# BillyXYB/TransEditor

Measured on AMD Instinct MI355X. Metric: 256x256 images/sec/GPU, G+D fwd+bwd, batch 16; 1/2/4/8-GPU scaling, higher is better.
Workload: dtype f32

## Files before the change

include/te_hip.h:

```cpp
#ifndef TE_HIP_H
#define TE_HIP_H

#include <stdint.h>

#ifdef __cplusplus
extern "C" {
#endif

#define TE_ABI_VERSION 3

#define TE_ERR_NULL -1
#define TE_ERR_SHAPE -2
#define TE_ERR_UNSUPPORTED -3
#define TE_ERR_WORKSPACE -4

typedef void* te_stream_t;

int te_version(void);
const char* te_last_error_string(void);
const char* te_arch(void);

int te_bias_act_f32(float* out, const float* x, const float* b, const float* ref, int act, int grad,
                    float alpha, float scale, int64_t size_x, int64_t step_b, int64_t size_b,
                    te_stream_t stream);
// ... 130 lines not shown
                             const float* residual, int I, int J, int K, int64_t sai, int64_t sak, int64_t sbk, int64_t sbj,
                             float alpha, float beta, int act, te_stream_t stream);

int te_minibatch_stddev_fwd_f32(float* y, const float* x, int B, int group, int C, int HW, float eps, te_stream_t stream);
int te_minibatch_stddev_bwd_f32(float* gx, const float* gy, const float* x, int B, int group, int C, int HW, float eps,
                                te_stream_t stream);

int te_layer_norm_supported(int64_t R, int N);
int te_layer_norm_fwd_f32(float* y, float* stats, const float* x, int64_t R, int N, float eps, te_stream_t stream);
int te_layer_norm_bwd_f32(float* gx, const float* g, const float* y, const float* stats, int64_t R, int N, te_stream_t stream);

int te_pixel_norm_supported(int64_t B, int D, int C);
int te_pixel_norm_fwd_f32(float* y, float* r, const float* x, int64_t B, int D, int C, float eps, te_stream_t stream);
int te_pixel_norm_bwd_f32(float* gx, const float* g, const float* y, const float* r, int64_t B, int D, int C, te_stream_t stream);

int te_small_gemm_batched_f32(float* c, const float* a, const float* b, const float* bias, int nz, int64_t za, int64_t zc,
                              int64_t zb, int64_t zbias, const int64_t* b_tab, const int64_t* bias_tab, int I, int J, int K,
                              int64_t sai, int64_t sak, int64_t sbk, int64_t sbj, int64_t sci, int64_t scj, float alpha,
                              float beta, int act, te_stream_t stream);

int te_demod_fwd_f32(float* d, float* wsq, const float* w, const float* s, float wscale, float eps, int B, int Co, int Ci,
                     int T, te_stream_t stream);
int te_demod_bwd_f32(float* gw, float* gs, const float* gd, const float* d, const float* w, const float* wsq,
                     const float* s, float wscale, int B, int Co, int Ci, int T, int accumulate, te_stream_t stream);

int te_mt_adam_f32(const int64_t* table, const int32_t* chunks, int n_tensors, int n_chunks, int chunk_elems, double lr,
                   double beta1, double beta2, double eps, int step, te_stream_t stream);
int te_mt_ema_f32(const int64_t* table, const int32_t* chunks, int n_tensors, int n_chunks, int chunk_elems, double decay,
                  te_stream_t stream);

int te_chan_scale_f32(float* out, const float* x, const float* s, int64_t rows, int64_t hw, te_stream_t stream);
int te_chan_dot_f32(float* out, const float* a, const float* b, int64_t rows, int64_t hw, te_stream_t stream);

int te_lpips_stem_fwd_f32(float* out, const float* x, const float* w, const float* b, int N, int H, int W, te_stream_t stream);
int te_lpips_stem_dgrad_f32(float* gx, const float* g, const float* y1, const float* w, int N, int H, int W, te_stream_t stream);
int te_maxpool2_fwd_f32(float* out, const float* x, int64_t planes, int H, int W, te_stream_t stream);
int te_maxpool2_bwd_f32(float* gx, const float* g, const float* x, int64_t planes, int H, int W, te_stream_t stream);
int te_lpips_normalize_f32(float* out, const float* x, int N, int C, int64_t HW, te_stream_t stream);
int te_lpips_head_blocks(int64_t HW);
int te_lpips_head_fwd_f32(float* partial, const float* f, const float* t, const float* w, int N, int Nt, int C, int64_t HW,
                          te_stream_t stream);
int te_lpips_dist_f32(float* d, const float* const* partial, const int64_t* hw, int L, int N, te_stream_t stream);
int te_lpips_head_bwd_f32(float* gf, const float* gin, const float* gd, const float* f, const float* t, const float* w, int N, int Nt,
                          int C, int64_t HW, int relu_mask, te_stream_t stream);
int te_lpips_pair_head_fwd_f32(float* partial, const float* f, const float* w, int N, int C, int64_t HW, te_stream_t stream);
int te_crop_resize_bilinear_f32(float* out, const float* img, int B, int H, int W, int y0, int x0, int hc, int wc, int h, int w,
                                te_stream_t stream);

int64_t te_noise_reg_ws_floats(const int* sizes, int n, int B);
int te_noise_reg_fwd_f32(float* loss, float* ws, float* const* maps, const int* sizes, int n, int B, te_stream_t stream);
int te_noise_reg_bwd_f32(float* const* grads, float* tws, const float* gloss, const float* ws, float* const* maps, const int* sizes,
                         int n, int B, te_stream_t stream);
int te_noise_normalize_f32(float* const* maps, const int* sizes, int n, int B, te_stream_t stream);

int64_t te_prdc_ws_bytes(int N, int M, int D, int k);
int te_row_sqnorm_f32(float* out, const float* x, int N, int D, te_stream_t stream);
int te_prdc_knn_f32(float* r2, const float* x, const float* nx, int N, int D, int k, void* ws, te_stream_t stream);
int te_prdc_counts_f32(int32_t* col_count, int32_t* row_any, float* row_min, const float* x, const float* nx, const float* rr2,
                       const float* y, const float* ny, const float* rf2, int N, int M, int D, void* ws, te_stream_t stream);

int te_vgg_stem_fwd_f32(float* out, const float* x, const float* w, const float* b, int N, int H, int W, te_stream_t stream);
int te_adaptive_avgpool_f32(float* out, const float* x, int64_t planes, int H, int W, int OH, int OW, te_stream_t stream);
int te_fc_stream_splits(int J, int K);
int64_t te_fc_stream_ws_bytes(int64_t I, int J, int K);
int te_fc_stream_f32(float* c, float* ws, const float* a, const float* w, const float* bias, int64_t I, int J, int K, int act,
                     te_stream_t stream);
// ... 20 lines not shown
```

transeditor_amd/_lib.py:

```python
import ctypes as C
import os

import torch

_HERE = os.path.dirname(os.path.abspath(__file__))
LIB_PATH = os.path.join(_HERE, 'libte_hip.so')
_lib = None

CONV_3X3, CONV_T2, CONV_S2, CONV_1X1, CONV_3X3W, CONV_3X3W6, CONV_S2S6, CONV_T2S6, CONV_1X1S6 = 0, 1, 2, 3, 4, 5, 6, 7, 8
(PACK_FWD, PACK_DGRAD, PACK_SWAP, PACK_WFWD, PACK_WDGRAD, PACK_W6FWD, PACK_W6DGRAD, PACK_S6FWD, PACK_S6SWAP, PACK_T6FWD,
 PACK_T6SWAP, PACK_P6FWD, PACK_P6DGRAD) = range(13)

_P, _I, _L, _F = C.c_void_p, C.c_int, C.c_int64, C.c_float
_SIGNATURES = {
    'te_version': (C.c_int, []),
    'te_last_error_string': (C.c_char_p, []),
    'te_arch': (C.c_char_p, []),
    'te_bias_act_f32': (C.c_int, [_P, _P, _P, _P, _I, _I, _F, _F, _L, _L, _L, _P]),
    'te_bias_act_f16': (C.c_int, [_P, _P, _P, _P, _I, _I, _F, _F, _L, _L, _L, _P]),
    'te_bias_act_f64': (C.c_int, [_P, _P, _P, _P, _I, _I, _F, _F, _L, _L, _L, _P]),
    'te_bias_act_bwd_ws_floats': (C.c_int64, [_L, _L, _L]),
    'te_bias_act_bwd_f32': (C.c_int, [_P, _P, _P, _P, _P, _F, _F, _L, _L, _L, _P]),
    'te_bias_act_bwd_rgb_supported': (C.c_int, [_L, _L, _L]),
    'te_bias_act_bwd_rgb_f32': (C.c_int, [_P, _P, _P, _P, _P, _P, _P, _P, _F, _F, _F, _L, _L, _L, _P]),
# ... 29 lines not shown
    'te_wgrad_group_f32': (C.c_int, [_P, _P, _P, _I, _I, _I, _I, _I, _I, _I, _I, _P]),
    'te_wgrad_reduce_ws_floats': (C.c_int64, [_I, _I, _I, _I, _I, _I, _I, _I]),
    'te_wgrad_reduce_f32': (C.c_int, [_P, _P, _P, _P, _P, _P, _F, _P, _P, _I, _I, _I, _I, _I, _P]),
    'te_rgb_supported': (C.c_int, [_I, _I, _I]),
    'te_rgb_fwd_f32': (C.c_int, [_P, _P, _P, _P, _P, _F, _I, _I, _I, _P]),
    'te_rgb_dgrad_f32': (C.c_int, [_P, _P, _P, _P, _F, _I, _I, _I, _P]),
    'te_rgb_wgrad_sum_f32': (C.c_int, [_P, _P, _P, _I, _I, _I, _I, _P]),
    'te_rgb_expand_f32': (C.c_int, [_P, _P, _P, _P, _I, _F, _I, _I, _I, _P]),
    'te_rgb_wgrad_slab_count': (C.c_int, [_I, _I, _I]),
    'te_rgb_wgrad_f32': (C.c_int, [_P, _P, _P, _I, _I, _I, _I, _P]),
    'te_blur_actgrad_tiles': (C.c_int, [_I] * 8),
    'te_blur_actgrad_f32': (C.c_int, [_P, _P, _P, _P, _P, _L, _I, _I, _I, _I, _I, _I, _I, _I, _F, _F, _P]),
    'te_blur_gradact_f32': (C.c_int, [_P, _P, _P, _P, _P, _L, _I, _I, _I, _I, _I, _I, _I, _I, _F, _F, _P]),
    'te_small_gemm_f32': (C.c_int, [_P, _P, _P, _P, _P, _P, _P, _F, _I, _I, _I, _L, _L, _L, _L, _F, _F, _I, _P]),
    'te_small_gemm_batched_f32': (C.c_int, [_P, _P, _P, _P, _I, _L, _L, _L, _L, _P, _P, _I, _I, _I, _L, _L, _L, _L, _L, _L,
                                             _F, _F, _I, _P]),
    'te_layer_norm_supported': (C.c_int, [_L, _I]),
    'te_layer_norm_fwd_f32': (C.c_int, [_P, _P, _P, _L, _I, _F, _P]),
    'te_layer_norm_bwd_f32': (C.c_int, [_P, _P, _P, _P, _L, _I, _P]),
    'te_pixel_norm_supported': (C.c_int, [_L, _I, _I]),
    'te_pixel_norm_fwd_f32': (C.c_int, [_P, _P, _P, _L, _I, _I, _F, _P]),
    'te_pixel_norm_bwd_f32': (C.c_int, [_P, _P, _P, _P, _L, _I, _I, _P]),
    'te_demod_fwd_f32': (C.c_int, [_P, _P, _P, _P, _F, _F, _I, _I, _I, _I, _P]),
    'te_demod_bwd_f32': (C.c_int, [_P, _P, _P, _P, _P, _P, _P, _F, _I, _I, _I, _I, _I, _P]),
    'te_attn_fwd_f32': (C.c_int, [_P, _P, _P, _P, _P, _F, _I, _I, _I, _I, _I, _P]),
    'te_attn_bwd_f32': (C.c_int, [_P, _P, _P, _P, _P, _P, _P, _P, _P, _F, _I, _I, _I, _I, _I, _P]),
    'te_small_gemm_splitk_f32': (C.c_int, [_P, _P, _P, _I, _P, _P, _P, _P, _I, _I, _I, _L, _L, _L, _L, _F, _F, _I, _P]),
    'te_minibatch_stddev_fwd_f32': (C.c_int, [_P, _P, _I, _I, _I, _I, _F, _P]),
    'te_minibatch_stddev_bwd_f32': (C.c_int, [_P, _P, _P, _I, _I, _I, _I, _F, _P]),
    'te_mt_adam_f32': (C.c_int, [_P, _P, _I, _I, _I, C.c_double, C.c_double, C.c_double, C.c_double, _I, _P]),
    'te_mt_ema_f32': (C.c_int, [_P, _P, _I, _I, _I, C.c_double, _P]),
    'te_chan_scale_f32': (C.c_int, [_P, _P, _P, _L, _L, _P]),
    'te_chan_dot_f32': (C.c_int, [_P, _P, _P, _L, _L, _P]),
    'te_lpips_stem_fwd_f32': (C.c_int, [_P, _P, _P, _P, _I, _I, _I, _P]),
    'te_lpips_stem_dgrad_f32': (C.c_int, [_P, _P, _P, _P, _I, _I, _I, _P]),
    'te_maxpool2_fwd_f32': (C.c_int, [_P, _P, _L, _I, _I, _P]),
    'te_maxpool2_bwd_f32': (C.c_int, [_P, _P, _P, _L, _I, _I, _P]),
    'te_lpips_normalize_f32': (C.c_int, [_P, _P, _I, _I, _L, _P]),
    'te_lpips_head_blocks': (C.c_int, [_L]),
    'te_lpips_head_fwd_f32': (C.c_int, [_P, _P, _P, _P, _I, _I, _I, _L, _P]),
    'te_lpips_dist_f32': (C.c_int, [_P, _P, _P, _I, _I, _P]),
    'te_lpips_head_bwd_f32': (C.c_int, [_P, _P, _P, _P, _P, _P, _I, _I, _I, _L, _I, _P]),
    'te_lpips_pair_head_fwd_f32': (C.c_int, [_P, _P, _P, _I, _I, _L, _P]),
    'te_crop_resize_bilinear_f32': (C.c_int, [_P, _P, _I, _I, _I, _I, _I, _I, _I, _I, _I, _P]),
    'te_noise_reg_ws_floats': (C.c_int64, [_P, _I, _I]),
    'te_noise_reg_fwd_f32': (C.c_int, [_P, _P, _P, _P, _I, _I, _P]),
    'te_noise_reg_bwd_f32': (C.c_int, [_P, _P, _P, _P, _P, _P, _I, _I, _P]),
    'te_noise_normalize_f32': (C.c_int, [_P, _P, _I, _I, _P]),
    'te_prdc_ws_bytes': (C.c_int64, [_I, _I, _I, _I]),
    'te_row_sqnorm_f32': (C.c_int, [_P, _P, _I, _I, _P]),
    'te_prdc_knn_f32': (C.c_int, [_P, _P, _P, _I, _I, _I, _P, _P]),
    'te_prdc_counts_f32': (C.c_int, [_P, _P, _P, _P, _P, _P, _P, _P, _P, _I, _I, _I, _P, _P]),
    'te_vgg_stem_fwd_f32': (C.c_int, [_P, _P, _P, _P, _I, _I, _I, _P]),
    'te_adaptive_avgpool_f32': (C.c_int, [_P, _P, _L, _I, _I, _I, _I, _P]),
    'te_fc_stream_splits': (C.c_int, [_I, _I]),
    'te_fc_stream_ws_bytes': (C.c_int64, [_L, _I, _I]),
    'te_fc_stream_f32': (C.c_int, [_P, _P, _P, _P, _P, _L, _I, _I, _I, _P]),
    'te_fid_moments_ws_bytes': (C.c_int64, [_L, _I]),
    'te_fid_moments_f64': (C.c_int, [_P, _P, _P, _P, _L, _I, _I, _P]),
    'te_fid_finalize_f64': (C.c_int, [_P, _P, _P, _P, _L, _I, _P]),
    'te_gram_f32': (C.c_int, [_P, _P, _I, _I, _P]),
    'te_svm_smo_f64': (C.c_int, [_P, _P, _P, _P, _P, _I, C.c_double, C.c_double, _L, _P]),
    'te_svm_coef_f32': (C.c_int, [_P, _P, _P, _P, _I, _I, _P]),
    'te_conv2d_f32': (C.c_int, [_P, _P, _P, _P] + [_I] * 13 + [_P]),
    'te_pool3_f32': (C.c_int, [_P, _P, _I, _I, _I, _I, _I, _I, _I, _P]),
    'te_resize_bilinear_f32': (C.c_int, [_P, _P, _L, _I, _I, _I, _I, _P]),
# ... 546 lines not shown
                                 _ptr(gsim.contiguous()) if gsim is not None else None, _ptr(q), _ptr(k), _ptr(v),
                                 _ptr(sim), scale, N, groups, M, L, Cn // groups, _stream()), 'te_attn_bwd_f32')
    return gq, gk, gv


def mt_adam(table, chunks, n_tensors, n_chunks, chunk_elems, lr, beta1, beta2, eps, step):
    _on_current_device(table)
    _check(lib().te_mt_adam_f32(table.data_ptr(), chunks.data_ptr(), n_tensors, n_chunks, chunk_elems, lr, beta1, beta2, eps,
                                step, _stream()), 'te_mt_adam_f32')


def mt_ema(table, chunks, n_tensors, n_chunks, chunk_elems, decay):
    _on_current_device(table)
    _check(lib().te_mt_ema_f32(table.data_ptr(), chunks.data_ptr(), n_tensors, n_chunks, chunk_elems, float(decay), _stream()),
           'te_mt_ema_f32')


def chan_scale(x, s):
    x, s = x.contiguous(), s.contiguous()
    rows = x.shape[0] * x.shape[1]
    out = torch.empty_like(x)
    _check(lib().te_chan_scale_f32(_ptr(out), _ptr(x), _ptr(s), rows, x.numel() // max(rows, 1), _stream()), 'te_chan_scale_f32')
    return out


def chan_dot(a, b):
    a, b = a.contiguous(), b.contiguous()
    rows = a.shape[0] * a.shape[1]
    out = torch.empty(a.shape[0], a.shape[1], device=a.device, dtype=a.dtype)
    _check(lib().te_chan_dot_f32(_ptr(out), _ptr(a), _ptr(b), rows, a.numel() // max(rows, 1), _stream()), 'te_chan_dot_f32')
    return out


def lpips_stem_fwd(x, w, b):
    x = x.contiguous()
    N, _, H, W = x.shape
    out = torch.empty(N, 64, H, W, device=x.device, dtype=x.dtype)
    _check(lib().te_lpips_stem_fwd_f32(_ptr(out), _ptr(x), _ptr(w), _ptr(b), N, H, W, _stream()), 'te_lpips_stem_fwd_f32')
    return out


def lpips_stem_dgrad(g, y1, w):
    g = g.contiguous()
    N, _, H, W = g.shape
    gx = torch.empty(N, 3, H, W, device=g.device, dtype=g.dtype)
    _check(lib().te_lpips_stem_dgrad_f32(_ptr(gx), _ptr(g), _ptr(y1), _ptr(w), N, H, W, _stream()), 'te_lpips_stem_dgrad_f32')
    return gx


def maxpool2_fwd(x):
    x = x.contiguous()
    N, Cn, H, W = x.shape
    out = torch.empty(N, Cn, H // 2, W // 2, device=x.device, dtype=x.dtype)
    _check(lib().te_maxpool2_fwd_f32(_ptr(out), _ptr(x), N * Cn, H, W, _stream()), 'te_maxpool2_fwd_f32')
    return out


def maxpool2_bwd(g, x):
    g = g.contiguous()
    N, Cn, H, W = x.shape
    gx = torch.empty_like(x)
    _check(lib().te_maxpool2_bwd_f32(_ptr(gx), _ptr(g), _ptr(x), N * Cn, H, W, _stream()), 'te_maxpool2_bwd_f32')
    return gx


def lpips_normalize(x):
# ... 269 lines not shown
    out = _slice_out(out, c0, B, Co, max(Ho, 0), max(Wo, 0), x, 'conv2d')
    _check(lib().te_conv2d_f32(_ptr(out), _ptr(x), _ptr(w), _ptr(bias), B, Ci, Co, H, W, kh, kw, stride, pad[0], pad[1], out.shape[1],
                               c0, act, _stream()), 'te_conv2d_f32')
    return out


def pool3(x, mode, out=None, c0=0):
    if x.ndim != 4:
        raise RuntimeError(f'te_hip: pool3 expects [B,C,H,W], got {tuple(x.shape)}')
    B, Cn, H, W = x.shape
    Ho, Wo = ((H - 3) // 2 + 1, (W - 3) // 2 + 1) if mode == POOL3_MAX_S2 else (H, W)
    out = _slice_out(out, c0, B, Cn, max(Ho, 0), max(Wo, 0), x, 'pool3')
    _check(lib().te_pool3_f32(_ptr(out), _ptr(x), B, Cn, H, W, mode, out.shape[1], c0, _stream()), 'te_pool3_f32')
    return out


def resize_bilinear(x, OH, OW):
    if x.ndim != 4:
        raise RuntimeError(f'te_hip: resize_bilinear expects [B,C,H,W], got {tuple(x.shape)}')
    x = x.contiguous()
    B, Cn, H, W = x.shape
    out = torch.empty(B, Cn, OH, OW, device=x.device, dtype=x.dtype)
    _check(lib().te_resize_bilinear_f32(_ptr(out), _ptr(x), B * Cn, H, W, OH, OW, _stream()), 'te_resize_bilinear_f32')
    return out


def _install_roctx():
    import functools
    import torch.cuda.nvtx as nvtx
    names = ['bias_act', 'bias_act_bwd', 'upfirdn2d_raw', 'blur_actgrad', 'blur_gradact', 'conv_pack', 'conv_pack2', 'conv_pack_multi', 'conv',
             'wgrad_slabs', 'wgrad_reduce', 'rgb_fwd', 'rgb_dgrad', 'rgb_expand', 'rgb_wgrad_slabs', 'small_gemm',
             'small_gemm_splitk', 'small_gemm_batched', 'minibatch_stddev_fwd', 'minibatch_stddev_bwd',
             'layer_norm_fwd', 'layer_norm_bwd', 'pixel_norm_fwd', 'pixel_norm_bwd', 'demod_fwd', 'demod_from_wsq', 'demod_bwd',
             'attn_fwd', 'attn_bwd', 'mt_adam', 'mt_ema', 'chan_scale', 'chan_dot', 'lpips_stem_fwd', 'lpips_stem_dgrad',
             'maxpool2_fwd', 'maxpool2_bwd', 'lpips_normalize', 'lpips_head_fwd', 'lpips_dist', 'lpips_head_bwd', 'lpips_pair_head_fwd', 'crop_resize_bilinear', 'noise_reg_fwd',
             'noise_reg_bwd', 'noise_normalize_', 'row_sqnorm', 'prdc_knn', 'prdc_counts', 'vgg_stem_fwd', 'adaptive_avgpool', 'fc_stream',
             'fid_moments', 'fid_finalize', 'gram', 'svm_smo', 'svm_coef', 'conv2d', 'pool3', 'resize_bilinear']
    g = globals()

    def wrap(fn, name):
        @functools.wraps(fn)
        def run(*a, **k):
            t = next((x for x in a if torch.is_tensor(x)), None)
            nvtx.range_push(f'te:{name} {tuple(t.shape)}' if t is not None else f'te:{name}')
            try:
                return fn(*a, **k)
            finally:
                nvtx.range_pop()
        return run
    for n in names:
        if n in g:
            g[n] = wrap(g[n], n)


ROCTX = os.environ.get('TE_ROCTX') == '1'
if ROCTX:
    _install_roctx()
```

transeditor_amd/csrc/chanscale.hip:

```cpp
#include "te_common.h"

namespace {

__global__ __launch_bounds__(256) void chan_scale_vec4_kernel(float4* __restrict__ out, const float4* __restrict__ x,
                                                              const float* __restrict__ s, int64_t n4, uint32_t hw4) {
    const int64_t stride = (int64_t)gridDim.x * blockDim.x;
    for (int64_t i = (int64_t)blockIdx.x * blockDim.x + threadIdx.x; i < n4; i += stride) {
        const float sc = s[i / hw4];
        float4 v = x[i];
        v.x *= sc; v.y *= sc; v.z *= sc; v.w *= sc;
        out[i] = v;
    }
}

__global__ __launch_bounds__(256) void chan_scale_flat4_kernel(float4* __restrict__ out, const float4* __restrict__ x,
                                                               const float* __restrict__ s, int64_t n4, int64_t hw) {
    const int64_t stride = (int64_t)gridDim.x * blockDim.x;
    for (int64_t i = (int64_t)blockIdx.x * blockDim.x + threadIdx.x; i < n4; i += stride) {
        const int64_t e = 4 * i, r = e / hw;
        const int left = (int)(hw - (e - r * hw));
        const float s0 = s[r], s1 = left < 4 ? s[r + 1] : s0;
        float4 v = x[i];
        v.x *= s0;
        v.y *= left > 1 ? s0 : s1;
// ... 31 lines not shown
        const float4* b4 = reinterpret_cast<const float4*>(br);
        const int64_t n4 = hw / 4;
        float c0 = 0.f, c1 = 0.f, c2 = 0.f, c3 = 0.f;
        int64_t j = tid;
        for (; j + 768 < n4; j += 1024) {
            const float4 u0 = a4[j], u1 = a4[j + 256], u2 = a4[j + 512], u3 = a4[j + 768];
            const float4 v0 = b4[j], v1 = b4[j + 256], v2 = b4[j + 512], v3 = b4[j + 768];
            c0 += u0.x * v0.x + u0.y * v0.y + u0.z * v0.z + u0.w * v0.w;
            c1 += u1.x * v1.x + u1.y * v1.y + u1.z * v1.z + u1.w * v1.w;
            c2 += u2.x * v2.x + u2.y * v2.y + u2.z * v2.z + u2.w * v2.w;
            c3 += u3.x * v3.x + u3.y * v3.y + u3.z * v3.z + u3.w * v3.w;
        }
        for (; j < n4; j += 256) {
            const float4 u = a4[j], v = b4[j];
            c0 += u.x * v.x + u.y * v.y + u.z * v.z + u.w * v.w;
        }
        acc = (c0 + c1) + (c2 + c3);
    } else {
        float c0 = 0.f, c1 = 0.f;
        int64_t j = tid;
        for (; j + 256 < hw; j += 512) { c0 += ar[j] * br[j]; c1 += ar[j + 256] * br[j + 256]; }
        for (; j < hw; j += 256) c0 += ar[j] * br[j];
        acc = c0 + c1;
    }
#pragma unroll
    for (int off = 32; off > 0; off >>= 1) acc += __shfl_down(acc, off, 64);
    if (lane == 0) part[wid] = acc;
    __syncthreads();
    if (tid == 0) out[r] = (part[0] + part[1]) + (part[2] + part[3]);
}

inline bool aligned16(const void* p) { return (reinterpret_cast<uintptr_t>(p) & 15) == 0; }

}

extern "C" int te_chan_scale_f32(float* out, const float* x, const float* s, int64_t rows, int64_t hw, te_stream_t stream_) {
    TE_REQUIRE(out && x && s, TE_ERR_NULL, "te_chan_scale_f32: NULL pointer");
    TE_REQUIRE(rows >= 0 && hw > 0, TE_ERR_SHAPE, "te_chan_scale_f32: bad dims");
    if (rows == 0) return 0;
    hipStream_t st = (hipStream_t)stream_;
    const int64_t n = rows * hw;
    if (hw % 4 == 0 && aligned16(out) && aligned16(x) && hw / 4 < (int64_t)0xFFFFFFFF) {
        const int grid = (int)std::min<int64_t>(te::cdiv(n / 4, 256), te::kNumCU * 16);
        chan_scale_vec4_kernel<<<grid, 256, 0, st>>>((float4*)out, (const float4*)x, s, n / 4, (uint32_t)(hw / 4));
    } else if (hw >= 4 && n >= 1024 && aligned16(out) && aligned16(x)) {
        const int grid = (int)std::min<int64_t>(te::cdiv(n / 4, 256), te::kNumCU * 16);
        chan_scale_flat4_kernel<<<grid, 256, 0, st>>>((float4*)out, (const float4*)x, s, n / 4, hw);
        if (n % 4) chan_scale_kernel<<<1, 64, 0, st>>>(out, x, s, n, hw, n - n % 4);
    } else {
        const int grid = (int)std::min<int64_t>(te::cdiv(n, 256), te::kNumCU * 16);
        chan_scale_kernel<<<grid, 256, 0, st>>>(out, x, s, n, hw, 0);
    }
    return te::launch_status("te_chan_scale_f32");
}

extern "C" int te_chan_dot_f32(float* out, const float* a, const float* b, int64_t rows, int64_t hw, te_stream_t stream_) {
    TE_REQUIRE(out && a && b, TE_ERR_NULL, "te_chan_dot_f32: NULL pointer");
    TE_REQUIRE(rows >= 0 && hw > 0 && rows < (int64_t)0x7FFFFFFF, TE_ERR_SHAPE, "te_chan_dot_f32: bad dims");
    if (rows == 0) return 0;
    const int vec = (hw % 4 == 0 && aligned16(a) && aligned16(b)) ? 1 : 0;
    const int64_t blocks = hw <= 64 ? te::cdiv(rows, 4) : rows;
    chan_dot_kernel<<<(unsigned)blocks, 256, 0, (hipStream_t)stream_>>>(out, a, b, rows, hw, vec);
    return te::launch_status("te_chan_dot_f32");
}
```

transeditor_amd/op/modconv.py:

```python
import contextlib

import os

import torch
from torch.autograd import Function

from .. import _lib
from .chanscale import chan_scale
from .fused_act import fused_leaky_relu

import threading


class _Graph:
    __slots__ = ('skip_w',)

    def __init__(self):
        self.skip_w = False


_DEFAULT_GRAPH = _Graph()


class _Local(threading.local):
# ... 352 lines not shown

    @staticmethod
    def backward(ctx, ggw):
        gy, x = ctx.saved_tensors
        with cache_of(ctx):
            g_gy = _ConvFwd.apply(x, ggw, ctx.kind, ctx.wscale) if ctx.needs_input_grad[0] else None
            g_x = _ConvDgrad.apply(gy, ggw, ctx.kind, ctx.wscale) if ctx.needs_input_grad[1] else None
        return g_gy, g_x, None, None, None


def set_split_bf16(on):
    on = bool(on)
    globals()['USE_SPLIT_BF16'] = on
    _lib.wgrad_split(int(on))
    return on


def conv_core(x, w, kind='3x3', wscale=1.0):
    return _ConvFwd.apply(x, w, kind, float(wscale))


_SCALE_FLOOR = 1e-20


def _nonzero(s):
    if s is None:
        return None
    return _Floor.apply(s)


class _Floor(Function):
    @staticmethod
    def forward(ctx, s):
        return torch.where(s.abs() < _SCALE_FLOOR, torch.where(s < 0, -_SCALE_FLOOR, _SCALE_FLOOR).to(s.dtype), s)

    @staticmethod
    def backward(ctx, g):
        return g


def _rgb_ok(w, d, x_like, kind):
    return (kind == '1x1' and d is None and w.shape[0] == 3
            and _lib.rgb_supported(3, w.shape[1], x_like.shape[2] * x_like.shape[3]))


def _chan_dot(a, b):
    from .chanscale import _ChanDot
    return _ChanDot.apply(a.contiguous(), b.contiguous())


class _MCFwd(Function):
    @staticmethod
    def forward(ctx, x, w, s, d, kind, wscale):
        ctx.kind, ctx.wscale = kind, wscale
        ctx.graph = current_graph()
        keep_cache(ctx)
        if _rgb_ok(w, d, x, kind):
            y = _lib.rgb_fwd(x, w.reshape(3, w.shape[1]), s.contiguous(), None, wscale)
        else:
            y = _fwd_raw(x, w, kind, s.contiguous(), None if d is None else d.contiguous(), None, 0, wscale)
        ctx.save_for_backward(x, w, s, d, y)
        return y

    @staticmethod
    def backward(ctx, gy):
        x, w, s, d, y = ctx.saved_tensors
        need = ctx.needs_input_grad
        skip_w = ctx.graph.skip_w or _DEFAULT_GRAPH.skip_w
        with cache_of(ctx):
            gx = _MCDgrad.apply(gy, w, s, d, ctx.kind, ctx.wscale) if (need[0] or need[2]) else None
            gw = _MCWgrad.apply(gy, x, s, d, ctx.kind, w.shape[2], ctx.wscale) if (need[1] and not skip_w) else None
        gs = _chan_dot(gx, x) / s if need[2] else None
        gd = _chan_dot(gy, y) / d if (d is not None and need[3]) else None
        return (gx if need[0] else None), gw, gs, gd, None, None


class _MCDgrad(Function):
    @staticmethod
    def forward(ctx, gy, w, s, d, kind, wscale):
        ctx.kind, ctx.wscale = kind, wscale
        keep_cache(ctx)
        if _rgb_ok(w, d, gy, kind):
            gx = _lib.rgb_dgrad(gy, w.reshape(3, w.shape[1]), s.contiguous(), w.shape[1], wscale)
        else:
            gx = _dgrad_raw(gy, w, kind, isc=None if d is None else d.contiguous(), osc=s.contiguous(), wscale=wscale)
        ctx.save_for_backward(gy, w, s, d, gx)
        return gx

    @staticmethod
    def backward(ctx, ggx):
        gy, w, s, d, gx = ctx.saved_tensors
        need = ctx.needs_input_grad
        with cache_of(ctx):
            y2 = _MCFwd.apply(ggx, w, s, d, ctx.kind, ctx.wscale) if (need[0] or (d is not None and need[3])) else None
            gw = _MCWgrad.apply(gy, ggx, s, d, ctx.kind, w.shape[2], ctx.wscale) if need[1] else None
        gs = _chan_dot(ggx, gx) / s if need[2] else None
        gd = _chan_dot(gy, y2) / d if (d is not None and need[3]) else None
        return (y2 if need[0] else None), gw, gs, gd, None, None


class _MCWgrad(Function):
    @staticmethod
    def forward(ctx, gy, x, s, d, kind, ksize, wscale):
        ctx.kind, ctx.wscale = kind, wscale
        keep_cache(ctx)
        ctx.save_for_backward(gy, x, s, d)
        Co, Ci = gy.shape[1], x.shape[1]
        gyc, xc = gy.contiguous(), x.contiguous()
        if kind == '1x1' and d is None and Co == 3 and _lib.rgb_supported(3, Ci, x.shape[2] * x.shape[3]):
            slabs = _lib.rgb_wgrad_slabs(gyc, xc)
        else:
            slabs = _wgrad_raw(gyc, xc, kind)
        gw, _, _ = _lib.wgrad_reduce(slabs, slabs[0, 0], wscale, s.contiguous(), None if d is None else d.contiguous(), want_w=True)
        return gw.reshape(Co, Ci, ksize, ksize)

    @staticmethod
    def backward(ctx, ggw):
        gy, x, s, d = ctx.saved_tensors
        need = ctx.needs_input_grad
        with cache_of(ctx):
            y2 = _MCFwd.apply(x, ggw, s, d, ctx.kind, ctx.wscale) if (need[0] or (d is not None and need[3])) else None
            gx = _MCDgrad.apply(gy, ggw, s, d, ctx.kind, ctx.wscale) if (need[1] or need[2]) else None
        gs = _chan_dot(gx, x) / s if need[2] else None
        gd = _chan_dot(gy, y2) / d if (d is not None and need[3]) else None
        return (y2 if need[0] else None), (gx if need[1] else None), gs, gd, None, None, None


def _closed_ok(x):
    return x.is_cuda and x.dtype == torch.float32


USE_CLOSED_MODCONV = True


def modconv_closed(x, w, isc, osc, kind='3x3', wscale=1.0):
    return _MCFwd.apply(x, w, _nonzero(isc), _nonzero(osc), kind, float(wscale))


def _composite(x, w, isc, osc, bias, act, kind, wscale=1.0):
    if USE_CLOSED_MODCONV and isc is not None and kind in ('3x3', 'up', '1x1') and _closed_ok(x):
        y = modconv_closed(x, w, isc, osc, kind, wscale)
        if act:
            return fused_leaky_relu(y, bias, 0.2, _act_gain(act))
        return y if bias is None else y + bias[None, :, None, None]
    if isc is not None:
        x = chan_scale(x, isc)
    y = conv_core(x, w, kind, wscale)
    if osc is not None:
        y = chan_scale(y, osc)
    if act:
        return fused_leaky_relu(y, bias, 0.2, _act_gain(act))
    if bias is not None:
        y = y + bias[None, :, None, None]
    return y


class _ModConvFused(Function):
# ... 130 lines not shown
```

Measured before the change: 148.0.

## Fuse modconv scale-gradient channel dots and divides into batched kernels

Adds a multi-job channel dot-and-divide kernel, a channel axpy kernel and a scale-floor kernel. The modulated-conv backward now computes the input-scale and demod-scale gradients in one launch instead of separate chan_dot plus divide ops. A new _MCBwd autograd function handles the double-backward path (e.g. path-length or R1 regularisation) with fused axpy combinations. This is meant to cut kernel launches and elementwise passes, at the cost of more complex custom autograd code that could diverge numerically or in gradient correctness.

```diff
diff --git a/include/te_hip.h b/include/te_hip.h
--- a/include/te_hip.h
+++ b/include/te_hip.h
@@ -186,6 +186,13 @@
 int te_chan_scale_f32(float* out, const float* x, const float* s, int64_t rows, int64_t hw, te_stream_t stream);
 int te_chan_dot_f32(float* out, const float* a, const float* b, int64_t rows, int64_t hw, te_stream_t stream);
 
+int te_chan_dotdiv_multi_f32(int n, float* const* out, const float* const* a, const float* const* b, const float* const* scale,
+                             const float* const* m1, const float* const* m2, const int64_t* rows, const int64_t* hw,
+                             te_stream_t stream);
+int te_chan_axpy_f32(float* out, const float* base, int nterms, const float* const* t, const float* const* num,
+                     const float* const* den, int64_t rows, int64_t hw, te_stream_t stream);
+int te_scale_floor_f32(float* out, const float* s, int64_t n, float floor, te_stream_t stream);
+
 int te_lpips_stem_fwd_f32(float* out, const float* x, const float* w, const float* b, int N, int H, int W, te_stream_t stream);
 int te_lpips_stem_dgrad_f32(float* gx, const float* g, const float* y1, const float* w, int N, int H, int W, te_stream_t stream);
 int te_maxpool2_fwd_f32(float* out, const float* x, int64_t planes, int H, int W, te_stream_t stream);
diff --git a/transeditor_amd/_lib.py b/transeditor_amd/_lib.py
--- a/transeditor_amd/_lib.py
+++ b/transeditor_amd/_lib.py
@@ -85,6 +85,9 @@
     'te_mt_ema_f32': (C.c_int, [_P, _P, _I, _I, _I, C.c_double, _P]),
     'te_chan_scale_f32': (C.c_int, [_P, _P, _P, _L, _L, _P]),
     'te_chan_dot_f32': (C.c_int, [_P, _P, _P, _L, _L, _P]),
+    'te_chan_dotdiv_multi_f32': (C.c_int, [_I, _P, _P, _P, _P, _P, _P, _P, _P, _P]),
+    'te_chan_axpy_f32': (C.c_int, [_P, _P, _I, _P, _P, _P, _L, _L, _P]),
+    'te_scale_floor_f32': (C.c_int, [_P, _P, _L, _F, _P]),
     'te_lpips_stem_fwd_f32': (C.c_int, [_P, _P, _P, _P, _I, _I, _I, _P]),
     'te_lpips_stem_dgrad_f32': (C.c_int, [_P, _P, _P, _P, _I, _I, _I, _P]),
     'te_maxpool2_fwd_f32': (C.c_int, [_P, _P, _L, _I, _I, _P]),
@@ -697,6 +700,58 @@
     return out
 
 
+def chan_dotdiv_multi(jobs):
+    n = len(jobs)
+    if not n:
+        return []
+    keep, outs = [], []
+    for a, b, sc, m1, m2 in jobs:
+        if a.shape != b.shape or a.dim() < 2:
+            raise RuntimeError(f'te_hip: chan_dotdiv_multi needs two operands of one shape, got {tuple(a.shape)} and {tuple(b.shape)}')
+        for v in (sc, m1, m2):
+            if v is not None and tuple(v.shape) != tuple(a.shape[:2]):
+                raise RuntimeError(f'te_hip: chan_dotdiv_multi needs [B,C] row vectors, got {tuple(v.shape)} for {tuple(a.shape)}')
+        keep.append([None if v is None else v.contiguous() for v in (a, b, sc, m1, m2)])
+        outs.append(torch.empty(a.shape[0], a.shape[1], device=a.device, dtype=a.dtype))
+    tab = lambda vals: (C.c_void_p * n)(*vals)
+    rows = [k[0].shape[0] * k[0].shape[1] for k in keep]
+    _check(lib().te_chan_dotdiv_multi_f32(
+        n, tab([_ptr(o) for o in outs]), *[tab([_ptr(k[i]) for k in keep]) for i in range(5)],
+        (C.c_int64 * n)(*rows), (C.c_int64 * n)(*[k[0].numel() // max(r, 1) for k, r in zip(keep, rows)]), _stream()),
+        'te_chan_dotdiv_multi_f32')
+    return outs
+
+
+def chan_axpy(base, terms, out=None):
+    keep = [(t.contiguous(), num.contiguous(), None if den is None else den.contiguous()) for t, num, den in terms]
+    t0 = keep[0][0]
+    for t, num, den in keep:
+        if t.shape != t0.shape or tuple(num.shape) != tuple(t0.shape[:2]) or (den is not None and den.shape != num.shape):
+            raise RuntimeError('te_hip: chan_axpy needs terms of one shape [B,C,...] with [B,C] coefficients')
+    if base is not None:
+        if base.shape != t0.shape:
+            raise RuntimeError('te_hip: chan_axpy base and terms differ in shape')
+        if out is not base:
+            base = base.contiguous()
+    if out is None:
+        out = torch.empty_like(t0)
+    elif out is not base or any(t.data_ptr() == out.data_ptr() for t, _, _ in keep):
+        raise RuntimeError('te_hip: chan_axpy writes a new tensor or over its base, never over a term')
+    n = len(keep)
+    tab = lambda vals: (C.c_void_p * n)(*vals)
+    rows = t0.shape[0] * t0.shape[1]
+    _check(lib().te_chan_axpy_f32(_ptr(out), _ptr(base), n, tab([_ptr(k[0]) for k in keep]), tab([_ptr(k[1]) for k in keep]),
+                                  tab([_ptr(k[2]) for k in keep]), rows, t0.numel() // max(rows, 1), _stream()), 'te_chan_axpy_f32')
+    return out
+
+
+def scale_floor(s, floor):
+    s = s.contiguous()
+    out = torch.empty_like(s)
+    _check(lib().te_scale_floor_f32(_ptr(out), _ptr(s), s.numel(), float(floor), _stream()), 'te_scale_floor_f32')
+    return out
+
+
 def lpips_stem_fwd(x, w, b):
     x = x.contiguous()
     N, _, H, W = x.shape
@@ -1032,7 +1087,7 @@
              'wgrad_slabs', 'wgrad_reduce', 'rgb_fwd', 'rgb_dgrad', 'rgb_expand', 'rgb_wgrad_slabs', 'small_gemm',
              'small_gemm_splitk', 'small_gemm_batched', 'minibatch_stddev_fwd', 'minibatch_stddev_bwd',
              'layer_norm_fwd', 'layer_norm_bwd', 'pixel_norm_fwd', 'pixel_norm_bwd', 'demod_fwd', 'demod_from_wsq', 'demod_bwd',
-             'attn_fwd', 'attn_bwd', 'mt_adam', 'mt_ema', 'chan_scale', 'chan_dot', 'lpips_stem_fwd', 'lpips_stem_dgrad',
+             'attn_fwd', 'attn_bwd', 'mt_adam', 'mt_ema', 'chan_scale', 'chan_dot', 'chan_dotdiv_multi', 'chan_axpy', 'scale_floor', 'lpips_stem_fwd', 'lpips_stem_dgrad',
              'maxpool2_fwd', 'maxpool2_bwd', 'lpips_normalize', 'lpips_head_fwd', 'lpips_dist', 'lpips_head_bwd', 'lpips_pair_head_fwd', 'crop_resize_bilinear', 'noise_reg_fwd',
              'noise_reg_bwd', 'noise_normalize_', 'row_sqnorm', 'prdc_knn', 'prdc_counts', 'vgg_stem_fwd', 'adaptive_avgpool', 'fc_stream',
              'fid_moments', 'fid_finalize', 'gram', 'svm_smo', 'svm_coef', 'conv2d', 'pool3', 'resize_bilinear']
diff --git a/transeditor_amd/csrc/chanscale.hip b/transeditor_amd/csrc/chanscale.hip
--- a/transeditor_amd/csrc/chanscale.hip
+++ b/transeditor_amd/csrc/chanscale.hip
@@ -87,6 +87,228 @@
 
 inline bool aligned16(const void* p) { return (reinterpret_cast<uintptr_t>(p) & 15) == 0; }
 
+struct DotJob {
+    const float* a; const float* b;
+    const float* scale;
+    const float* m1; const float* m2;
+    float* out;
+    int64_t rows, hw;
+    int64_t blk0;
+};
+constexpr int DOT_MAXJOBS = 8;
+struct DotJobs { DotJob j[DOT_MAXJOBS]; int n; };
+
+__device__ inline float dot4(const float4 u, const float4 v) { return u.x * v.x + u.y * v.y + u.z * v.z + u.w * v.w; }
+
+__device__ inline void dot_store(const DotJob& J, int64_t r, float acc) {
+    if (J.m1) acc -= J.m1[r] * J.m2[r];
+    J.out[r] = J.scale ? acc / J.scale[r] : acc;
+}
+
+__global__ __launch_bounds__(256) void chan_dotdiv_multi_kernel(const DotJobs P) {
+    __shared__ float part[4];
+    int ji = 0;
+#pragma unroll
+    for (int q = 1; q < DOT_MAXJOBS; ++q)
+        if (q < P.n && (int64_t)blockIdx.x >= P.j[q].blk0) ji = q;
+    const DotJob J = P.j[ji];
+    const int64_t blk = (int64_t)blockIdx.x - J.blk0;
+    const int tid = threadIdx.x, lane = tid & 63, wid = tid >> 6;
+    const int64_t hw = J.hw;
+    if (hw <= 64) {
+        const int64_t r = blk * 4 + wid;
+        float acc = 0.f;
+        if (r < J.rows && lane < hw) acc = J.a[r * hw + lane] * J.b[r * hw + lane];
+#pragma unroll
+        for (int off = 32; off > 0; off >>= 1) acc += __shfl_down(acc, off, 64);
+        if (r < J.rows && lane == 0) dot_store(J, r, acc);
+        return;
+    }
+    const int64_t r = blk;
+    const float* ar = J.a + r * hw;
+    const float* br = J.b + r * hw;
+    const int ma = (int)((reinterpret_cast<uintptr_t>(ar) >> 2) & 3), mb = (int)((reinterpret_cast<uintptr_t>(br) >> 2) & 3);
+    float acc;
+    if (ma == mb) {
+        const int head = (4 - ma) & 3;
+        const int64_t n4 = (hw - head) / 4;
+        const int tail = (int)(hw - head - 4 * n4);
+        const float4* a4 = reinterpret_cast<const float4*>(ar + head);
+        const float4* b4 = reinterpret_cast<const float4*>(br + head);
+        float c0 = 0.f, c1 = 0.f, c2 = 0.f, c3 = 0.f;
+        int64_t j = tid;
+        for (; j + 768 < n4; j += 1024) {
+            const float4 u0 = a4[j], u1 = a4[j + 256], u2 = a4[j + 512], u3 = a4[j + 768];
+            const float4 v0 = b4[j], v1 = b4[j + 256], v2 = b4[j + 512], v3 = b4[j + 768];
+            c0 += dot4(u0, v0);
+            c1 += dot4(u1, v1);
+            c2 += dot4(u2, v2);
+            c3 += dot4(u3, v3);
+        }
+        for (; j < n4; j += 256) c0 += dot4(a4[j], b4[j]);
+        if (tid < head) c1 += ar[tid] * br[tid];
+        if (tid < tail) c2 += ar[head + 4 * n4 + tid] * br[head + 4 * n4 + tid];
+        acc = (c0 + c1) + (c2 + c3);
+    } else {
+        float c0 = 0.f, c1 = 0.f;
+        int64_t j = tid;
+        for (; j + 256 < hw; j += 512) { c0 += ar[j] * br[j]; c1 += ar[j + 256] * br[j + 256]; }
+        for (; j < hw; j += 256) c0 += ar[j] * br[j];
+        acc = c0 + c1;
+    }
+#pragma unroll
+    for (int off = 32; off > 0; off >>= 1) acc += __shfl_down(acc, off, 64);
+    if (lane == 0) part[wid] = acc;
+    __syncthreads();
+    if (tid == 0) dot_store(J, r, (part[0] + part[1]) + (part[2] + part[3]));
+}
+
+struct AxpyArgs {
+    float* out; const float* base;
+    const float* t[3]; const float* num[3]; const float* den[3];
+    int64_t n, hw;
+};
+
+template <int NT>
+__device__ inline void axpy_coef(const AxpyArgs& A, int64_t r, float (&c)[NT]) {
+#pragma unroll
+    for (int k = 0; k < NT; ++k) c[k] = A.den[k] ? A.num[k][r] / A.den[k][r] : A.num[k][r];
+}
+
+template <int NT, bool BASE, typename I>
+__global__ __launch_bounds__(256) void chan_axpy_flat4_kernel(const AxpyArgs A) {
+    const I n4 = (I)(A.n / 4), hw = (I)A.hw;
+    const I stride = (I)gridDim.x * 256;
+    const float4* b4 = reinterpret_cast<const float4*>(A.base);
+    float4* o4 = reinterpret_cast<float4*>(A.out);
+    for (I i = (I)blockIdx.x * 256 + threadIdx.x; i < n4; i += stride) {
+        const I e = 4 * i, r = e / hw;
+        const I left = hw - (e - r * hw);
+        float c0[NT], c1[NT];
+        axpy_coef<NT>(A, (int64_t)r, c0);
+        if (left < 4) axpy_coef<NT>(A, (int64_t)r + 1, c1);
+        else {
+#pragma unroll
+            for (int k = 0; k < NT; ++k) c1[k] = c0[k];
+        }
+        float4 v = make_float4(0.f, 0.f, 0.f, 0.f);
+        if (BASE) v = b4[i];
+#pragma unroll
+        for (int k = 0; k < NT; ++k) {
+            const float4 t = reinterpret_cast<const float4*>(A.t[k])[i];
+            v.x += c0[k] * t.x;
+            v.y += (left > 1 ? c0[k] : c1[k]) * t.y;
+            v.z += (left > 2 ? c0[k] : c1[k]) * t.z;
+            v.w += (left > 3 ? c0[k] : c1[k]) * t.w;
+        }
+        o4[i] = v;
+    }
+    const int rest = (int)(A.n & 3);
+    if (blockIdx.x == 0 && (int)threadIdx.x < rest) {
+        const int64_t i = A.n - rest + threadIdx.x;
+        float c[NT];
+        axpy_coef<NT>(A, i / A.hw, c);
+        float v = BASE ? A.base[i] : 0.f;
+#pragma unroll
+        for (int k = 0; k < NT; ++k) v += c[k] * A.t[k][i];
+        A.out[i] = v;
+    }
+}
+
+template <int NT, bool BASE>
+__global__ __launch_bounds__(256) void chan_axpy_kernel(const AxpyArgs A) {
+    const int64_t stride = (int64_t)gridDim.x * 256;
+    for (int64_t i = (int64_t)blockIdx.x * 256 + threadIdx.x; i < A.n; i += stride) {
+        float c[NT];
+        axpy_coef<NT>(A, i / A.hw, c);
+        float v = BASE ? A.base[i] : 0.f;
+#pragma unroll
+        for (int k = 0; k < NT; ++k) v += c[k] * A.t[k][i];
+        A.out[i] = v;
+    }
+}
+
+template <int NT, bool BASE>
+void axpy_launch(const AxpyArgs& A, bool vec, hipStream_t st) {
+    if (vec) {
+        const int grid = (int)std::min<int64_t>(te::cdiv(A.n / 4, 256), te::kNumCU * 16);
+        if (A.n < (int64_t)0x7FFFFFFF) chan_axpy_flat4_kernel<NT, BASE, uint32_t><<<grid, 256, 0, st>>>(A);
+        else chan_axpy_flat4_kernel<NT, BASE, int64_t><<<grid, 256, 0, st>>>(A);
+    } else {
+        const int grid = (int)std::min<int64_t>(te::cdiv(A.n, 256), te::kNumCU * 16);
+        chan_axpy_kernel<NT, BASE><<<grid, 256, 0, st>>>(A);
+    }
+}
+
+__global__ __launch_bounds__(256) void scale_floor_kernel(float* __restrict__ out, const float* __restrict__ s, int64_t n, float floor_) {
+    const int64_t i = (int64_t)blockIdx.x * 256 + threadIdx.x;
+    if (i < n) {
+        const float v = s[i];
+        out[i] = fabsf(v) < floor_ ? (v < 0.f ? -floor_ : floor_) : v;
+    }
+}
+
+}
+
+extern "C" int te_chan_dotdiv_multi_f32(int n, float* const* out, const float* const* a, const float* const* b,
+                                        const float* const* scale, const float* const* m1, const float* const* m2,
+                                        const int64_t* rows, const int64_t* hw, te_stream_t stream_) {
+    TE_REQUIRE(n >= 0 && (n == 0 || (out && a && b && rows && hw)), TE_ERR_NULL, "te_chan_dotdiv_multi_f32: NULL table");
+    for (int base = 0; base < n; base += DOT_MAXJOBS) {
+        const int cnt = std::min(DOT_MAXJOBS, n - base);
+        DotJobs P{};
+        int64_t blocks = 0;
+        for (int i = 0; i < cnt; ++i) {
+            const int e = base + i;
+            TE_REQUIRE(out[e] && a[e] && b[e], TE_ERR_NULL, "te_chan_dotdiv_multi_f32: NULL pointer in job %d", e);
+            TE_REQUIRE(rows[e] >= 0 && hw[e] > 0, TE_ERR_SHAPE, "te_chan_dotdiv_multi_f32: bad dims in job %d", e);
+            const float* mm1 = m1 ? m1[e] : nullptr;
+            const float* mm2 = m2 ? m2[e] : nullptr;
+            TE_REQUIRE((mm1 == nullptr) == (mm2 == nullptr), TE_ERR_NULL, "te_chan_dotdiv_multi_f32: job %d has one of m1 / m2 only", e);
+            P.j[i] = DotJob{a[e], b[e], scale ? scale[e] : nullptr, mm1, mm2, out[e], rows[e], hw[e], blocks};
+            blocks += hw[e] <= 64 ? te::cdiv(rows[e], 4) : rows[e];
+        }
+        P.n = cnt;
+        TE_REQUIRE(blocks < (int64_t)0x7FFFFFFF, TE_ERR_SHAPE, "te_chan_dotdiv_multi_f32: too many rows");
+        if (blocks == 0) continue;
+        chan_dotdiv_multi_kernel<<<(unsigned)blocks, 256, 0, (hipStream_t)stream_>>>(P);
+    }
+    return te::launch_status("te_chan_dotdiv_multi_f32");
+}
+
+extern "C" int te_chan_axpy_f32(float* out, const float* base, int nterms, const float* const* t, const float* const* num,
+                                const float* const* den, int64_t rows, int64_t hw, te_stream_t stream_) {
+    TE_REQUIRE(out && t && num, TE_ERR_NULL, "te_chan_axpy_f32: NULL pointer");
+    TE_REQUIRE(nterms >= 1 && nterms <= 3, TE_ERR_UNSUPPORTED, "te_chan_axpy_f32: 1 to 3 terms, got %d", nterms);
+    TE_REQUIRE(rows >= 0 && hw > 0, TE_ERR_SHAPE, "te_chan_axpy_f32: bad dims");
+    if (rows == 0) return 0;
+    AxpyArgs A{};
+    A.out = out; A.base = base; A.n = rows * hw; A.hw = hw;
+    bool vec = hw >= 4 && A.n >= 1024 && aligned16(out) && (!base || aligned16(base));
+    for (int k = 0; k < nterms; ++k) {
+        TE_REQUIRE(t[k] && num[k], TE_ERR_NULL, "te_chan_axpy_f32: NULL pointer in term %d", k);
+        A.t[k] = t[k]; A.num[k] = num[k]; A.den[k] = den ? den[k] : nullptr;
+        vec = vec && aligned16(t[k]);
+    }
+    hipStream_t st = (hipStream_t)stream_;
+    const int sel = nterms * 2 + (base ? 1 : 0);
+    switch (sel) {
+        case 2: axpy_launch<1, false>(A, vec, st); break;
+        case 3: axpy_launch<1, true>(A, vec, st); break;
+        case 4: axpy_launch<2, false>(A, vec, st); break;
+        case 5: axpy_launch<2, true>(A, vec, st); break;
+        case 6: axpy_launch<3, false>(A, vec, st); break;
+        default: axpy_launch<3, true>(A, vec, st); break;
+    }
+    return te::launch_status("te_chan_axpy_f32");
+}
+
+extern "C" int te_scale_floor_f32(float* out, const float* s, int64_t n, float floor_, te_stream_t stream_) {
+    TE_REQUIRE(out && s, TE_ERR_NULL, "te_scale_floor_f32: NULL pointer");
+    TE_REQUIRE(n >= 0 && floor_ > 0.f, TE_ERR_SHAPE, "te_scale_floor_f32: bad arguments");
+    if (n == 0) return 0;
+    scale_floor_kernel<<<(unsigned)te::cdiv(n, 256), 256, 0, (hipStream_t)stream_>>>(out, s, n, floor_);
+    return te::launch_status("te_scale_floor_f32");
 }
 
 extern "C" int te_chan_scale_f32(float* out, const float* x, const float* s, int64_t rows, int64_t hw, te_stream_t stream_) {
diff --git a/transeditor_amd/op/modconv.py b/transeditor_amd/op/modconv.py
--- a/transeditor_amd/op/modconv.py
+++ b/transeditor_amd/op/modconv.py
@@ -408,6 +408,8 @@
 class _Floor(Function):
     @staticmethod
     def forward(ctx, s):
+        if _merged_ok(s):
+            return _lib.scale_floor(s, _SCALE_FLOOR)
         return torch.where(s.abs() < _SCALE_FLOOR, torch.where(s < 0, -_SCALE_FLOOR, _SCALE_FLOOR).to(s.dtype), s)
 
     @staticmethod
@@ -423,6 +425,36 @@
 def _chan_dot(a, b):
     from .chanscale import _ChanDot
     return _ChanDot.apply(a.contiguous(), b.contiguous())
+
+
+USE_MERGED_SCALE_GRADS = True
+
+
+def _merged_ok(t):
+    from . import chanscale
+    return USE_MERGED_SCALE_GRADS and chanscale.USE_KERNELS and t.is_cuda and t.dtype == torch.float32
+
+
+def _scale_grads(*terms):
+    live = [t for t in terms if t is not None]
+    if not live:
+        return [None] * len(terms)
+    if torch.is_grad_enabled() or not _merged_ok(live[0][0]):
+        return [None if t is None else _chan_dot(t[0], t[1]) / t[2] for t in terms]
+    outs = iter(_lib.chan_dotdiv_multi([(a, b, sc, None, None) for a, b, sc in live]))
+    return [None if t is None else next(outs) for t in terms]
+
+
+def _mc_fwd_raw(x, w, s, d, kind, wscale):
+    if _rgb_ok(w, d, x, kind):
+        return _lib.rgb_fwd(x, w.reshape(3, w.shape[1]), s.contiguous(), None, wscale)
+    return _fwd_raw(x, w, kind, s.contiguous(), None if d is None else d.contiguous(), None, 0, wscale)
+
+
+def _mc_dgrad_raw(gy, w, s, d, kind, wscale):
+    if _rgb_ok(w, d, gy, kind):
+        return _lib.rgb_dgrad(gy, w.reshape(3, w.shape[1]), s.contiguous(), w.shape[1], wscale)
+    return _dgrad_raw(gy, w, kind, isc=None if d is None else d.contiguous(), osc=s.contiguous(), wscale=wscale)
 
 
 class _MCFwd(Function):
@@ -431,10 +463,7 @@
         ctx.kind, ctx.wscale = kind, wscale
         ctx.graph = current_graph()
         keep_cache(ctx)
-        if _rgb_ok(w, d, x, kind):
-            y = _lib.rgb_fwd(x, w.reshape(3, w.shape[1]), s.contiguous(), None, wscale)
-        else:
-            y = _fwd_raw(x, w, kind, s.contiguous(), None if d is None else d.contiguous(), None, 0, wscale)
+        y = _mc_fwd_raw(x, w, s, d, kind, wscale)
         ctx.save_for_backward(x, w, s, d, y)
         return y
 
@@ -443,12 +472,85 @@
         x, w, s, d, y = ctx.saved_tensors
         need = ctx.needs_input_grad
         skip_w = ctx.graph.skip_w or _DEFAULT_GRAPH.skip_w
+        want_gs, want_gd = need[2], d is not None and need[3]
         with cache_of(ctx):
-            gx = _MCDgrad.apply(gy, w, s, d, ctx.kind, ctx.wscale) if (need[0] or need[2]) else None
+            if torch.is_grad_enabled() and (want_gs or want_gd) and _merged_ok(gy):
+                gx, gs, gd = _MCBwd.apply(gy, x, y, w, s, d, ctx.kind, ctx.wscale, want_gs, want_gd)
+            else:
+                gx = _MCDgrad.apply(gy, w, s, d, ctx.kind, ctx.wscale) if (need[0] or need[2]) else None
+                gs, gd = _scale_grads((gx, x, s) if want_gs else None, (gy, y, d) if want_gd else None)
             gw = _MCWgrad.apply(gy, x, s, d, ctx.kind, w.shape[2], ctx.wscale) if (need[1] and not skip_w) else None
-        gs = _chan_dot(gx, x) / s if need[2] else None
-        gd = _chan_dot(gy, y) / d if (d is not None and need[3]) else None
         return (gx if need[0] else None), gw, gs, gd, None, None
+
+
+class _MCBwd(Function):
+    @staticmethod
+    def forward(ctx, gy, x, y, w, s, d, kind, wscale, want_gs, want_gd):
+        ctx.kind, ctx.wscale = kind, wscale
+        keep_cache(ctx)
+        ctx.set_materialize_grads(False)
+        gx = _mc_dgrad_raw(gy, w, s, d, kind, wscale)
+        jobs = ([(gx, x, s, None, None)] if want_gs else []) + ([(gy, y, d, None, None)] if want_gd else [])
+        outs = iter(_lib.chan_dotdiv_multi(jobs))
+        gs = next(outs) if want_gs else None
+        gd = next(outs) if want_gd else None
+        ctx.save_for_backward(gy, x, y, w, s, d, gx, gs, gd)
+        return gx, gs, gd
+
+    @staticmethod
+    def backward(ctx, ggx, cs, cd):
+        if torch.is_grad_enabled():
+            return _MCBwd._recorded(ctx, ggx, cs, cd)
+        gy, x, y, w, s, d, gx, gs, gd = ctx.saved_tensors
+        need = ctx.needs_input_grad
+        kind, wscale = ctx.kind, ctx.wscale
+        need_d = d is not None and need[5]
+        G = ggx if cs is None else _lib.chan_axpy(ggx, [(x, cs, s)])
+        y2 = gw = g_s = g_d = g_gy = g_x = g_y = None
+        if G is not None:
+            with cache_of(ctx):
+                if need[0] or need_d:
+                    y2 = _mc_fwd_raw(G, w, s, d, kind, wscale)
+                if need[3]:
+                    gw = _MCWgrad.apply(gy, G, s, d, kind, w.shape[2], wscale)
+        jobs = []
+        if need[4] and ggx is not None:
+            jobs.append((ggx, gx, s, None, None))
+        if need_d and y2 is not None:
+            jobs.append((gy, y2, d, cd, None if cd is None else gd))
+        outs = iter(_lib.chan_dotdiv_multi(jobs))
+        if need[4] and ggx is not None:
+            g_s = next(outs)
+        if need_d:
+            g_d = next(outs) if y2 is not None else (None if cd is None else -(cd * gd / d))
+        if need[0]:
+            g_gy = y2 if cd is None else _lib.chan_axpy(y2, [(y, cd, d)], out=y2)
+        if need[1] and cs is not None:
+            g_x = _lib.chan_axpy(None, [(gx, cs, s)])
+        if need[2] and cd is not None:
+            g_y = _lib.chan_axpy(None, [(gy, cd, d)])
+        return g_gy, g_x, g_y, gw, g_s, g_d, None, None, None, None
+
+    @staticmethod
+    def _recorded(ctx, ggx, cs, cd):
+        gy, x, y, w, s, d = ctx.saved_tensors[:6]
+        need = ctx.needs_input_grad
+        with torch.enable_grad(), cache_of(ctx):
+            al = [None if t is None else t.view_as(t) for t in (gy, x, y, w, s, d)]
+            a_gy, a_x, a_y, a_w, a_s, a_d = al
+            gx = _MCDgrad.apply(a_gy, a_w, a_s, a_d, ctx.kind, ctx.wscale)
+            outs, cots = [], []
+            if ggx is not None:
+                outs.append(gx); cots.append(ggx)
+            if cs is not None:
+                outs.append(_chan_dot(gx, a_x) / a_s); cots.append(cs)
+            if cd is not None:
+                outs.append(_chan_dot(a_gy, a_y) / a_d); cots.append(cd)
+            ins = [t for t, n in zip(al, need[:6]) if n and t is not None]
+            if not outs or not ins:
+                return (None,) * 10
+            gr = iter(torch.autograd.grad(outs, ins, cots, create_graph=True, allow_unused=True))
+        return tuple(next(gr) if (n and t is not None) else None for t, n in zip(al, need[:6])) + (None,) * 4
 
 
 class _MCDgrad(Function):
@@ -456,10 +558,7 @@
     def forward(ctx, gy, w, s, d, kind, wscale):
         ctx.kind, ctx.wscale = kind, wscale
         keep_cache(ctx)
-        if _rgb_ok(w, d, gy, kind):
-            gx = _lib.rgb_dgrad(gy, w.reshape(3, w.shape[1]), s.contiguous(), w.shape[1], wscale)
-        else:
-            gx = _dgrad_raw(gy, w, kind, isc=None if d is None else d.contiguous(), osc=s.contiguous(), wscale=wscale)
+        gx = _mc_dgrad_raw(gy, w, s, d, kind, wscale)
         ctx.save_for_backward(gy, w, s, d, gx)
         return gx
 
@@ -467,11 +566,11 @@
     def backward(ctx, ggx):
         gy, w, s, d, gx = ctx.saved_tensors
         need = ctx.needs_input_grad
+        need_d = d is not None and need[3]
         with cache_of(ctx):
-            y2 = _MCFwd.apply(ggx, w, s, d, ctx.kind, ctx.wscale) if (need[0] or (d is not None and need[3])) else None
+            y2 = _MCFwd.apply(ggx, w, s, d, ctx.kind, ctx.wscale) if (need[0] or need_d) else None
             gw = _MCWgrad.apply(gy, ggx, s, d, ctx.kind, w.shape[2], ctx.wscale) if need[1] else None
-        gs = _chan_dot(ggx, gx) / s if need[2] else None
-        gd = _chan_dot(gy, y2) / d if (d is not None and need[3]) else None
+        gs, gd = _scale_grads((ggx, gx, s) if need[2] else None, (gy, y2, d) if need_d else None)
         return (y2 if need[0] else None), gw, gs, gd, None, None
 
 
@@ -494,11 +593,11 @@
     def backward(ctx, ggw):
         gy, x, s, d = ctx.saved_tensors
         need = ctx.needs_input_grad
+        need_d = d is not None and need[3]
         with cache_of(ctx):
-            y2 = _MCFwd.apply(x, ggw, s, d, ctx.kind, ctx.wscale) if (need[0] or (d is not None and need[3])) else None
+            y2 = _MCFwd.apply(x, ggw, s, d, ctx.kind, ctx.wscale) if (need[0] or need_d) else None
             gx = _MCDgrad.apply(gy, ggw, s, d, ctx.kind, ctx.wscale) if (need[1] or need[2]) else None
-        gs = _chan_dot(gx, x) / s if need[2] else None
-        gd = _chan_dot(gy, y2) / d if (d is not None and need[3]) else None
+        gs, gd = _scale_grads((gx, x, s) if need[2] else None, (gy, y2, d) if need_d else None)
         return (y2 if need[0] else None), (gx if need[1] else None), gs, gd, None, None, None
 
 
```

Result: no change. 148.5, median of 6 (+0.3%).
